# zju3dv/PVO

Hardware: AMD Instinct MI355X
Metric: VO keyframe updates/sec (8-keyframe window, 512x384, 36 edges; 6 graph updates + edge rebuild per keyframe) (higher is better)
Workload: dtype f16 (volume, lookup, update operator) / f32 (BA assembly) / f64 (pose solve); 1 GPU; S-B: BASELINE.json configs[1] window (8 keyframes, 48x64 maps, E=36, itrs=2), synthetic; edges=36, parallelism=independent window per GPU

## Files before the change

pvo_amd/csrc/conv_small.hip:

```cpp
#include "operand16.h"
#include <type_traits>
#include "glo_tile.h"
#include <stdlib.h>

namespace {

constexpr int kTH = 8, kTW = 16, kR = 3;
#ifndef PVO_CONV7_ROWS
#define PVO_CONV7_ROWS 16
#endif
constexpr int kTH7 = PVO_CONV7_ROWS;
constexpr int kHW_ = kTW + 2 * kR, kHH7 = kTH7 + 2 * kR;
constexpr int kTaps = 49, kSteps = 13;

template <typename T>
__global__ __launch_bounds__(256) void conv7x7_c8_kernel(const uint16_t* __restrict__ x, const uint16_t* __restrict__ wt,
                                                         const float* __restrict__ bias, uint16_t* __restrict__ y,
                                                         int H, int W) {
  __shared__ __attribute__((aligned(16))) unsigned char halo[kHH7 * kHW_ * 16];
  __shared__ __attribute__((aligned(16))) unsigned char slab[2][16 * 272];
  const int e = blockIdx.z, y0 = blockIdx.y * kTH7, x0 = blockIdx.x * kTW;
  const int tid = threadIdx.x, lane = tid & 63;
  const int wave = __builtin_amdgcn_readfirstlane(tid >> 6);
  const int li = lane & 15, lk = lane >> 4;
// ... 97 lines not shown
#pragma unroll
    for (int nt = 0; nt < NT; ++nt) bcur[kc][nt] = *reinterpret_cast<const u32x4*>(wl + static_cast<size_t>(nt) * 16 * 128 + kc * 32);
  v4f acc[kTH][NT];
#pragma unroll
  for (int py = 0; py < kTH; ++py)
#pragma unroll
    for (int nt = 0; nt < NT; ++nt) acc[py][nt] = v4f{0.f, 0.f, 0.f, 0.f};
  __syncthreads();

#pragma unroll 1
  for (int t = 0; t < 9; ++t) {
    if (t < 8) {
#pragma unroll
      for (int kc = 0; kc < 4; ++kc)
#pragma unroll
        for (int nt = 0; nt < NT; ++nt)
          bnxt[kc][nt] = *reinterpret_cast<const u32x4*>(wl + (t + 1) * tap_stride + static_cast<size_t>(nt) * 16 * 128 + kc * 32);
    }
    const unsigned char* tp = c3s + ((t / 3) * (kTW + 2) + (t % 3) + li) * kC3Stride + lk * 16;
#pragma unroll
    for (int py = 0; py < kTH; ++py) {
#pragma unroll
      for (int kc = 0; kc < 4; ++kc) {
        const u32x4 a = *reinterpret_cast<const u32x4*>(tp + py * (kTW + 2) * kC3Stride + kc * 64);
#pragma unroll
        for (int nt = 0; nt < NT; ++nt) acc[py][nt] = pvo_mfma<T>(a, bcur[kc][nt], acc[py][nt]);
      }
    }
    if (t < 8) {
#pragma unroll
      for (int kc = 0; kc < 4; ++kc)
#pragma unroll
        for (int nt = 0; nt < NT; ++nt) bcur[kc][nt] = bnxt[kc][nt];
    }
  }
  __syncthreads();
  constexpr int kOutStride = kCoutWG * 2 + 16;
  float bb[NT];
#pragma unroll
  for (int nt = 0; nt < NT; ++nt) bb[nt] = bias ? bias[co0 + nt * 16 + li] : 0.0f;
#pragma unroll
  for (int py = 0; py < kTH; ++py)
#pragma unroll
    for (int nt = 0; nt < NT; ++nt)
#pragma unroll
      for (int r = 0; r < 4; ++r) {
        float v = acc[py][nt][r] + bb[nt];
        if (relu) v = fmaxf(v, 0.0f);
        *reinterpret_cast<uint16_t*>(c3s + (py * 16 + lk * 4 + r) * kOutStride + (wave * 16 * NT + nt * 16 + li) * 2) =
            static_cast<uint16_t>(pvo_bits<T>(v));
      }
  __syncthreads();
  constexpr int kChunks = kCoutWG / 8;
  for (int id = tid; id < kTH * 16 * kChunks; id += 256) {
    const int p = id / kChunks, c = id - p * kChunks;
    const int gy = y0 + (p >> 4), gx = x0 + (p & 15);
    if (gy < H && gx < W)
      *reinterpret_cast<u32x4*>(y + ((static_cast<size_t>(e) * H + gy) * W + gx) * ystride + yoff + cg * kCoutWG + c * 8) =
          *reinterpret_cast<const u32x4*>(c3s + p * kOutStride + c * 16);
  }
}


struct BigEpi {
  int mode;
  const float* g;
  const uint16_t* P;
  const int* p_slots;
  const uint16_t* net;
  const uint16_t* Z;
  uint16_t* y2;
  int nseg;
  const uint16_t* seg_p[3]; int seg_stride[3]; int seg_chunks[3];
  const uint16_t* w2f;
  float* z;
};

constexpr int kBT = 16;
constexpr int kBHalo = (kBT + 2) * (kBT + 2);
constexpr int kBPitch = kBT + 2;
constexpr int kBStride = 96;
constexpr int kBA = 384 * kBStride;
constexpr int kBLds = 2 * kBA;

__device__ __forceinline__ int big_pix(int mt, int q) { return (q >> 1) * 16 + 2 * mt + (q & 1); }

#ifdef PVO_CONV_PROBE
__device__ unsigned long long* g_conv_probe = nullptr;
#define CONV_WG ((static_cast<size_t>(blockIdx.z) * gridDim.y + blockIdx.y) * gridDim.x + blockIdx.x)
#define CONV_PROBE(slot)                                                                                          \
  do {                                                                                                            \
    if (g_conv_probe && threadIdx.x == 0) g_conv_probe[CONV_WG * 8 + (slot)] = __builtin_readcyclecounter();      \
  } while (0)
#else
#define CONV_PROBE(slot)
#endif

template <typename T, bool HEADS>
__global__ __launch_bounds__(256, 2) void conv3x3_big_kernel(const uint16_t* __restrict__ x, const uint16_t* __restrict__ wt,
                                                          const float* __restrict__ bias, uint16_t* __restrict__ y,
                                                          int H, int W, int Cin, int Cout, int relu, int ystride, int yoff, BigEpi ep) {
  extern __shared__ __attribute__((aligned(16))) unsigned char bs[];
  unsigned char* As = bs;
  CONV_PROBE(0);
#ifdef PVO_CONV_PROBE
  if (g_conv_probe && threadIdx.x == 0) {
    g_conv_probe[CONV_WG * 8 + 4] = (static_cast<unsigned long long>(__builtin_amdgcn_s_getreg(20 | (31 << 11))) << 32) | __builtin_amdgcn_s_getreg(4 | (31 << 11));
    g_conv_probe[CONV_WG * 8 + 5] = wall_clock64();
  }
#endif
  const int ntx = (W + kBT - 1) / kBT;
  const int cg = blockIdx.x / ntx, tx_ = blockIdx.x - cg * ntx;
  const int e = blockIdx.z, y0 = blockIdx.y * kBT, x0 = tx_ * kBT;
  const int tid = threadIdx.x, lane = tid & 63;
  const int wave = __builtin_amdgcn_readfirstlane(tid >> 6);
  const int wm = wave >> 1, wn = wave & 1;
  const int li = lane & 15, kg = lane >> 4;
  const int nC = Cin >> 5;
  const uint16_t* xe = x + static_cast<size_t>(e) * H * W * Cin;

  u32x4 ra[3];
  int apix[6];
#pragma unroll
  for (int it = 0; it < 6; ++it) {
    const int id = tid + 256 * it;
    const int pos = id >> 2;
    apix[it] = -1;
    if (pos < kBHalo) {
      const int hr = pos / (kBT + 2), hc = pos % (kBT + 2);
      const int hy = y0 - 1 + hr, hx = x0 - 1 + hc;
      if (hy >= 0 && hy < H && hx >= 0 && hx < W) apix[it] = hy * W + hx;
    }
  }
  const int lpos0 = (tid >> 2) * kBStride + (tid & 3) * 16;
  auto lpos = [&](int it) { return lpos0 + it * 64 * kBStride; };
  const size_t img = static_cast<size_t>(e) * H * W;
  const uint16_t* a_src = xe; int a_stride = Cin, a_coff = 0;
  auto select_a = [&](int cc) {
    a_src = xe; a_stride = Cin; a_coff = cc * 32;
    if (ep.nseg > 0) {
      int sgi = 0, c0 = cc;
      while (sgi + 1 < ep.nseg && c0 >= ep.seg_chunks[sgi]) { c0 -= ep.seg_chunks[sgi]; ++sgi; }
      a_stride = ep.seg_stride[sgi];
      a_src = ep.seg_p[sgi] + img * a_stride;
      a_coff = c0 * 32;
    }
  };
  auto fetch_a = [&](int half) {
#pragma unroll
    for (int k = 0; k < 3; ++k)
      ra[k] = *reinterpret_cast<const u32x4*>(a_src + static_cast<size_t>(max(apix[3 * half + k], 0)) * a_stride + a_coff + (tid & 3) * 8);
  };
  auto store_a = [&](int buf, int half) {
#pragma unroll
    for (int k = 0; k < 3; ++k) {
      u32x4 v = ra[k];
      if (apix[3 * half + k] < 0) v = u32x4{0u, 0u, 0u, 0u};
      *reinterpret_cast<u32x4*>(As + buf * kBA + lpos(3 * half + k)) = v;
    }
  };

  float ginit[4] = {0.0f, 0.0f, 0.0f, 0.0f};
  if (!HEADS && ep.mode != 0) {
#pragma unroll
    for (int nt = 0; nt < 4; ++nt)
      ginit[nt] = ep.g[static_cast<size_t>(e) * 384 + (ep.mode == 1 ? cg * 128 : 256) + wn * 64 + nt * 16 + li];
  }
  v4f acc[8][4];
#pragma unroll
  for (int mt = 0; mt < 8; ++mt)
#pragma unroll
    for (int nt = 0; nt < 4; ++nt)
#pragma unroll
      for (int r = 0; r < 4; ++r) acc[mt][nt][r] = ginit[nt];

  const int S = nC * 9;
  {
    const uint16_t* wf = wt + (static_cast<size_t>(cg) * S * 8 + wn * 4) * 512;
    const int lane_off = lane * 8;
    u32x4 bset[3][4];
    auto fetch_bf = [&](u32x4 (&r)[4], int s) {
      const uint16_t* p = wf + static_cast<size_t>(min(s, S - 1)) * 4096;
#pragma unroll
      for (int f = 0; f < 4; ++f) r[f] = *reinterpret_cast<const u32x4*>(p + lane_off + f * 512);
    };
    select_a(0);
    {
      u32x4 r6[6];
#pragma unroll
      for (int k = 0; k < 6; ++k)
        r6[k] = *reinterpret_cast<const u32x4*>(a_src + static_cast<size_t>(max(apix[k], 0)) * a_stride + a_coff + (tid & 3) * 8);
      fetch_bf(bset[0], 0); fetch_bf(bset[1], 1);
#pragma unroll
      for (int k = 0; k < 6; ++k) {
        u32x4 v = r6[k];
        if (apix[k] < 0) v = u32x4{0u, 0u, 0u, 0u};
        *reinterpret_cast<u32x4*>(As + lpos(k)) = v;
      }
    }
    __syncthreads();
    CONV_PROBE(1);
    const unsigned char* Abase = As + ((8 * wm + (li >> 1)) * kBPitch + (li & 1)) * kBStride + kg * 16;
    auto main_loop = [&](auto nh_c) {
    constexpr int NH = decltype(nh_c)::value;
    auto read_half = [&](u32x4 (&a)[4], const unsigned char* Ac, int toff, int h) {
#pragma unroll
      for (int i = 0; i < 4; ++i) a[i] = *reinterpret_cast<const u32x4*>(Ac + toff + (4 * h + i) * 2 * kBStride);
    };
    auto mfma_half = [&](const u32x4 (&a)[4], const u32x4 (&bf)[4], int h, bool n_major) {
#pragma unroll
      for (int j = 0; j < 16; ++j) {
        const int i = n_major ? (j & 3) : (j >> 2), nt = n_major ? (j >> 2) : (j & 3);
        acc[4 * h + i][nt] = pvo_mfma<T>(a[i], bf[nt], acc[4 * h + i][nt]);
      }
    };
    auto pin_reads_b = [&]() {
#pragma unroll
      for (int i = 0; i < 4; ++i) {
        __builtin_amdgcn_sched_group_barrier(0x8, 1, 0); __builtin_amdgcn_sched_group_barrier(0x100, 1, 0);
        __builtin_amdgcn_sched_group_barrier(0x8, 1, 0); __builtin_amdgcn_sched_group_barrier(0x20, 1, 0);
      }
    };
    auto pin_reads = [&]() {
#pragma unroll
      for (int i = 0; i < 4; ++i) { __builtin_amdgcn_sched_group_barrier(0x8, 2, 0); __builtin_amdgcn_sched_group_barrier(0x100, 1, 0); }
    };
    auto pin_staging = [&](int t) {
      if (t == 3 || t == 7) {
#pragma unroll
        for (int i = 0; i < 3; ++i) { __builtin_amdgcn_sched_group_barrier(0x8, 1, 0); __builtin_amdgcn_sched_group_barrier(0x200, 1, 0); }
      }
      if (t == 3) { __builtin_amdgcn_sched_group_barrier(0x8, 1, 0); __builtin_amdgcn_sched_group_barrier(0x20, 3, 0); }
    };
#pragma unroll 1
    for (int cc = 0; cc < nC; ++cc) {
      const unsigned char* Ac = Abase + (cc & 1) * kBA;
      select_a(min(cc + 1, nC - 1));
      fetch_a(0);
      u32x4 a0[4], a1[4];
      read_half(a0, Ac, 0, 0);
      __builtin_amdgcn_sched_barrier(0);
#pragma unroll
      for (int t = 0; t < 9; ++t) {
        const int toff = ((t / 3) * kBPitch + (t % 3)) * kBStride;
        const int toff1 = (((t + 1) / 3) * kBPitch + ((t + 1) % 3)) * kBStride;
        fetch_bf(bset[(t + 2) % 3], cc * 9 + t + 2);
        const u32x4 (&bf)[4] = bset[t % 3];
        if (NH == 2) {
          read_half(a1, Ac, toff, 1);
          mfma_half(a0, bf, 0, false);
          pin_reads_b();
          __builtin_amdgcn_sched_barrier(0);
          if (t < 8) read_half(a0, Ac, toff1, 0);
          if (t == 3) { store_a((cc + 1) & 1, 0); fetch_a(1); }
          if (t == 7) store_a((cc + 1) & 1, 1);
          mfma_half(a1, bf, 1, true);
          if (t < 8) pin_reads();
          pin_staging(t);
        } else {
          u32x4 (&cur)[4] = (t & 1) ? a1 : a0;
          u32x4 (&nxt)[4] = (t & 1) ? a0 : a1;
          if (t < 8) read_half(nxt, Ac, toff1, 0);
          if (t == 3) { store_a((cc + 1) & 1, 0); fetch_a(1); }
          if (t == 7) store_a((cc + 1) & 1, 1);
          mfma_half(cur, bf, 0, true);
          if (t < 8) pin_reads_b();
          else {
#pragma unroll
            for (int i = 0; i < 4; ++i) { __builtin_amdgcn_sched_group_barrier(0x8, 1, 0); __builtin_amdgcn_sched_group_barrier(0x20, 1, 0); }
          }
          pin_staging(t);
        }
        __builtin_amdgcn_sched_barrier(0);
      }
      __syncthreads();
    }
    };
    if (x0 + 8 >= W) main_loop(std::integral_constant<int, 1>{});
    else main_loop(std::integral_constant<int, 2>{});
  }
  CONV_PROBE(2);

  if (!HEADS && ep.mode != 0) {
    float* slab = reinterpret_cast<float*>(bs);
    const int c = tid & 15, m0 = tid >> 4;
    const int pstride = ep.mode == 1 ? 256 : 128;
    const uint16_t* gate_p = ep.P + (ep.mode == 1 ? cg * 128 : 0) + c * 8;
    uint16_t* const dst = (ep.mode == 1 && cg != 0) ? ep.y2 : y;
    const int ep_ = ep.p_slots ? ep.p_slots[e] : e;
    u32x4 pv[4], nv[4], zv[4];
    auto request = [&](int half, int b) {
#pragma unroll
      for (int k = 0; k < 4; ++k) {
        const int m = m0 + 16 * (4 * b + k);
        const int gy = y0 + 8 * half + (m >> 4), gx = x0 + (m & 15);
        const bool in = gy < H && gx < W;
        const size_t rr = in ? (static_cast<size_t>(e) * H + gy) * W + gx : 0;
        const size_t rp = in ? (static_cast<size_t>(ep_) * H + gy) * W + gx : 0;
        pv[k] = *reinterpret_cast<const u32x4*>(gate_p + rp * pstride);
        nv[k] = *reinterpret_cast<const u32x4*>(ep.net + rr * 128 + c * 8);
        if (ep.mode == 2) zv[k] = *reinterpret_cast<const u32x4*>(ep.Z + rr * 128 + c * 8);
      }
    };
    auto finish = [&](int half, int b) {
#pragma unroll
      for (int k = 0; k < 4; ++k) {
        const int m = m0 + 16 * (4 * b + k);
        const int gy = y0 + 8 * half + (m >> 4), gx = x0 + (m & 15);
        float a[8], pp[8], nn[8], o[8];
        const float4 a0 = *reinterpret_cast<const float4*>(slab + m * 132 + c * 8), a1 = *reinterpret_cast<const float4*>(slab + m * 132 + c * 8 + 4);
        a[0] = a0.x; a[1] = a0.y; a[2] = a0.z; a[3] = a0.w; a[4] = a1.x; a[5] = a1.y; a[6] = a1.z; a[7] = a1.w;
        pvo_unpack8<T>(pv[k], pp);
        pvo_unpack8<T>(nv[k], nn);
        if (ep.mode == 1) {
#pragma unroll
          for (int q = 0; q < 8; ++q) o[q] = __builtin_amdgcn_rcpf(1.0f + __builtin_amdgcn_exp2f(-1.4426950408889634f * (a[q] + pp[q])));
          if (cg != 0) {
#pragma unroll
            for (int q = 0; q < 8; ++q) o[q] *= nn[q];
          }
        } else {
          float zz[8];
          pvo_unpack8<T>(zv[k], zz);
#pragma unroll
          for (int q = 0; q < 8; ++q) {
            const float th = 1.0f - 2.0f * __builtin_amdgcn_rcpf(1.0f + __builtin_amdgcn_exp2f(2.8853900817779268f * (a[q] + pp[q])));
            o[q] = (1.0f - zz[q]) * nn[q] + zz[q] * th;
          }
        }
        if (gy < H && gx < W) *reinterpret_cast<u32x4*>(dst + ((static_cast<size_t>(e) * H + gy) * W + gx) * 128 + c * 8) = pvo_pack8<T>(o);
      }
    };
#pragma unroll 1
    for (int half = 0; half < 2; ++half) {
      request(half, 0);
      if (wm == half) {
#pragma unroll
        for (int mt = 0; mt < 8; ++mt)
#pragma unroll
          for (int nt = 0; nt < 4; ++nt)
#pragma unroll
            for (int r = 0; r < 4; ++r) slab[big_pix(mt, 4 * kg + r) * 132 + wn * 64 + nt * 16 + li] = acc[mt][nt][r];
      }
      __syncthreads();
      if (half == 0) CONV_PROBE(6);
      finish(half, 0);
      request(half, 1);
      finish(half, 1);
      __syncthreads();
      if (half == 0) CONV_PROBE(7);
    }
    CONV_PROBE(3);
    return;
  }
  float bb[4];
#pragma unroll
  for (int nt = 0; nt < 4; ++nt) bb[nt] = bias ? bias[cg * 128 + wn * 64 + nt * 16 + li] : 0.0f;
  unsigned char* w2s = bs + 36 * 1024;
  if (HEADS) {
    const u32x4* src = reinterpret_cast<const u32x4*>(ep.w2f + static_cast<size_t>(cg) * 4096) + tid;
    const u32x4 f0 = src[0], f1 = src[256];
    *reinterpret_cast<u32x4*>(w2s + tid * 16) = f0;
    *reinterpret_cast<u32x4*>(w2s + 4096 + tid * 16) = f1;
  }
#pragma unroll 1
  for (int half = 0; half < 2; ++half) {
    if (wm == half) {
#pragma unroll
      for (int mt = 0; mt < 8; ++mt)
#pragma unroll
        for (int nt = 0; nt < 4; ++nt)
#pragma unroll
          for (int r = 0; r < 4; ++r) {
            const int m = big_pix(mt, 4 * kg + r);
            float v = acc[mt][nt][r] + bb[nt];
            if (relu) v = fmaxf(v, 0.0f);
            *reinterpret_cast<uint16_t*>(bs + m * 272 + (wn * 64 + nt * 16 + li) * 2) = static_cast<uint16_t>(pvo_bits<T>(v));
          }
    }
    __syncthreads();
    if (HEADS) {
      v16f zz;
#pragma unroll
      for (int r = 0; r < 16; ++r) zz[r] = 0.0f;
      const int l32 = lane & 31, k32 = lane >> 5;
      const unsigned char* arow = bs + (32 * wave + l32) * 272 + k32 * 16;
#pragma unroll
      for (int ks = 0; ks < 8; ++ks)
        zz = pvo_mfma32<T>(*reinterpret_cast<const u32x4*>(arow + ks * 32), *reinterpret_cast<const u32x4*>(w2s + (ks * 64 + lane) * 16), zz);
      if (l32 < 18) {
#pragma unroll
        for (int r = 0; r < 16; ++r) {
          const int m = 32 * wave + (r & 3) + 8 * (r >> 2) + 4 * k32;
          const int gy = y0 + 8 * half + (m >> 4), gx = x0 + (m & 15);
          if (gy < H && gx < W) ep.z[(((static_cast<size_t>(e) * H + gy) * W + gx) * (Cout >> 7) + cg) * 18 + l32] = zz[r];
        }
      }
    } else {
      for (int id = tid; id < 128 * 16; id += 256) {
        const int m = id >> 4, c = id & 15;
        const int gy = y0 + 8 * half + (m >> 4), gx = x0 + (m & 15);
        if (gy < H && gx < W)
          *reinterpret_cast<u32x4*>(y + ((static_cast<size_t>(e) * H + gy) * W + gx) * ystride + yoff + cg * 128 + c * 8) =
              *reinterpret_cast<const u32x4*>(bs + m * 272 + c * 16);
      }
    }
    __syncthreads();
  }
  CONV_PROBE(3);
}

constexpr int kFeOW = 14;
constexpr int kFeRows = kTH + 2;
constexpr int kFeM7W = 16 + 2 * kR;
constexpr int kFeM7Pos = (kFeRows + 2 * kR) * kFeM7W;
constexpr int kFeF1Pos = kFeRows * 16 + 2;
constexpr int kFeLds = kFeF1Pos * kC3Stride + kFeM7Pos * 16;

template <typename T>
__global__ __launch_bounds__(256) void flow_encoder_kernel(const uint16_t* __restrict__ x, const uint16_t* __restrict__ w7,
                                                           const float* __restrict__ b7, const uint16_t* __restrict__ w3,
                                                           const float* __restrict__ b3, uint16_t* __restrict__ y,
                                                           int H, int W, int ystride, int yoff) {
  extern __shared__ __attribute__((aligned(16))) unsigned char fes[];
  unsigned char* f1 = fes;
  unsigned char* halo = fes + kFeF1Pos * kC3Stride;
  const int e = blockIdx.z, y0 = blockIdx.y * kTH, x0 = blockIdx.x * kFeOW;
  const int tid = threadIdx.x, lane = tid & 63;
  const int wave = __builtin_amdgcn_readfirstlane(tid >> 6);
  const int li = lane & 15, lk = lane >> 4;

  {
    u32x4 bf[kSteps][2];
#pragma unroll
    for (int s = 0; s < kSteps; ++s)
#pragma unroll
      for (int nt = 0; nt < 2; ++nt)
        bf[s][nt] = *reinterpret_cast<const u32x4*>(w7 + (static_cast<size_t>(4 * s + lk) * 128 + wave * 32 + nt * 16 + li) * 8);
    const uint16_t* xe = x + static_cast<size_t>(e) * H * W * 8;
    for (int pos = tid; pos < kFeM7Pos; pos += 256) {
      const int hy = y0 - 1 - kR + pos / kFeM7W, hx = x0 - 1 - kR + pos % kFeM7W;
      u32x4 v = {0u, 0u, 0u, 0u};
      if (hy >= 0 && hy < H && hx >= 0 && hx < W) v = *reinterpret_cast<const u32x4*>(xe + (static_cast<size_t>(hy) * W + hx) * 8);
      *reinterpret_cast<u32x4*>(halo + pos * 16) = v;
    }
    if (tid < 2 * 17) *reinterpret_cast<u32x4*>(f1 + kFeRows * 16 * kC3Stride + tid * 16) = u32x4{0u, 0u, 0u, 0u};
    int toff[kSteps];
#pragma unroll
    for (int s = 0; s < kSteps; ++s) {
      const int tap = min(4 * s + lk, kTaps - 1);
      toff[s] = ((tap / 7) * kFeM7W + (tap % 7) + li) * 16;
    }
    const float bb0 = b7[wave * 32 + li], bb1 = b7[wave * 32 + 16 + li];
    __syncthreads();
    for (int r = 0; r < kFeRows; ++r) {
      const int gy = y0 - 1 + r;
      v4f d0 = {0.f, 0.f, 0.f, 0.f}, d1 = {0.f, 0.f, 0.f, 0.f};
      const bool row_in = gy >= 0 && gy < H;
      if (row_in) {
        const unsigned char* rowp = halo + r * kFeM7W * 16;
        u32x4 afr[kSteps];
#pragma unroll
        for (int s = 0; s < kSteps; ++s) afr[s] = *reinterpret_cast<const u32x4*>(rowp + toff[s]);
#pragma unroll
        for (int s = 0; s < kSteps; ++s) {
          d0 = pvo_mfma<T>(afr[s], bf[s][0], d0);
          d1 = pvo_mfma<T>(afr[s], bf[s][1], d1);
        }
      }
#pragma unroll
      for (int q = 0; q < 4; ++q) {
        const int p = lk * 4 + q, gx = x0 - 1 + p;
        const bool in = row_in && gx >= 0 && gx < W;
        unsigned char* dst = f1 + (r * 16 + p) * kC3Stride + (wave * 32 + li) * 2;
        *reinterpret_cast<uint16_t*>(dst) = in ? static_cast<uint16_t>(pvo_bits<T>(fmaxf(d0[q] + bb0, 0.0f))) : static_cast<uint16_t>(0);
        *reinterpret_cast<uint16_t*>(dst + 32) = in ? static_cast<uint16_t>(pvo_bits<T>(fmaxf(d1[q] + bb1, 0.0f))) : static_cast<uint16_t>(0);
      }
    }
  }
  const int co0 = wave * 16;
  const uint16_t* wl = w3 + (static_cast<size_t>(co0 + li)) * 128 + lk * 8;
  constexpr size_t tap_stride = static_cast<size_t>(64) * 128;
  u32x4 bcur[4], bnxt[4];
#pragma unroll
  for (int kc = 0; kc < 4; ++kc) bcur[kc] = *reinterpret_cast<const u32x4*>(wl + kc * 32);
  v4f acc[kTH];
#pragma unroll
  for (int py = 0; py < kTH; ++py) acc[py] = v4f{0.f, 0.f, 0.f, 0.f};
  __syncthreads();
#pragma unroll 1
// ... 62 lines not shown

extern "C" int pvo_flow_encoder(const void* x, const void* w7_taps, const float* bias7, const void* w3_taps, const float* bias3,
                                void* y, int E, int H, int W, int ystride, int yoff, int dtype, void* stream) {
  if (E < 0 || H < 0 || W < 0) return PVO_EINVAL;
  if (ystride == 0) ystride = 64;
  if (ystride < yoff + 64 || yoff < 0 || (ystride & 7) || (yoff & 7)) return PVO_EINVAL;
  if (E == 0 || H == 0 || W == 0) return PVO_OK;
  if (!x || !w7_taps || !bias7 || !w3_taps || !y || E > 65535) return PVO_EINVAL;
  if (pvo_misaligned16(x, w7_taps, w3_taps, y)) return PVO_EINVAL;
  hipStream_t st = pvo_stream(stream);
  const dim3 grid((W + kFeOW - 1) / kFeOW, (H + kTH - 1) / kTH, E);
  const uint16_t *xp = static_cast<const uint16_t*>(x), *w7 = static_cast<const uint16_t*>(w7_taps), *w3 = static_cast<const uint16_t*>(w3_taps);
  return pvo_dispatch16(dtype, [&](auto tag) -> int {
    using T = decltype(tag);
    if (!pvo_allow_lds<flow_encoder_kernel<T>>(kFeLds)) return PVO_ELAUNCH;
    hipLaunchKernelGGL(flow_encoder_kernel<T>, grid, dim3(256), kFeLds, st, xp, w7, bias7, w3, bias3, static_cast<uint16_t*>(y), H, W, ystride, yoff);
    PVO_CHECK_LAUNCH();
    return PVO_OK;
  });
}

extern "C" int pvo_gru_glo_chunks(int HW) { return HW <= 0 ? 0 : (HW + 255) / 256; }

extern "C" int pvo_gru_glo_fused(const void* net, const void* w_weight, const float* w_bias, float* glo_part,
                                 int E, int HW, int dtype, void* stream) {
  if (E < 0 || HW < 0) return PVO_EINVAL;
  if (E == 0 || HW == 0) return PVO_OK;
  if (!net || !w_weight || !glo_part || E > 65535) return PVO_EINVAL;
  if (pvo_misaligned16(net, w_weight)) return PVO_EINVAL;
  hipStream_t st = pvo_stream(stream);
  const int chunk = 256;
  dim3 grid(pvo_gru_glo_chunks(HW), E);
  return pvo_dispatch16(dtype, [&](auto tag) -> int {
    using T = decltype(tag);
    hipLaunchKernelGGL(gru_glo_mfma_kernel<T>, grid, dim3(256), 0, st, static_cast<const uint16_t*>(net),
                       static_cast<const uint16_t*>(w_weight), w_bias, glo_part, HW, chunk);
    PVO_CHECK_LAUNCH();
    return PVO_OK;
  });
}

extern "C" int pvo_conv3x3_c128(const void* x, const void* w_taps, const float* bias, void* y,
                                int E, int H, int W, int Cout, int relu, int ystride, int yoff, int dtype, void* stream) {
  if (E < 0 || H < 0 || W < 0) return PVO_EINVAL;
  if (Cout != 64 && (Cout <= 0 || (Cout & 127))) return PVO_EUNSUPPORTED;
  if (ystride == 0) ystride = Cout;
  if (ystride < yoff + Cout || yoff < 0 || (ystride & 7) || (yoff & 7)) return PVO_EINVAL;
  if (E == 0 || H == 0 || W == 0) return PVO_OK;
  if (!x || !w_taps || !y || E > 65535) return PVO_EINVAL;
  if (pvo_misaligned16(x, w_taps, y)) return PVO_EINVAL;
  hipStream_t st = pvo_stream(stream);
  const int ntx = (W + kTW - 1) / kTW;
  const size_t lds = static_cast<size_t>(kC3Halo) * kC3Stride;
  const uint16_t* xp = static_cast<const uint16_t*>(x);
  const uint16_t* wp = static_cast<const uint16_t*>(w_taps);
  uint16_t* yp = static_cast<uint16_t*>(y);
  return pvo_dispatch16(dtype, [&](auto tag) -> int {
    using T = decltype(tag);
    if (Cout == 64) {
      dim3 grid(ntx, (H + kTH - 1) / kTH, E);
      hipLaunchKernelGGL((conv3x3_c128_kernel<T, 1>), grid, dim3(256), lds, st, xp, wp, bias, yp, H, W, Cout, relu, ystride, yoff);
    } else {
      dim3 grid(ntx * (Cout / 128), (H + kTH - 1) / kTH, E);
      hipLaunchKernelGGL((conv3x3_c128_kernel<T, 2>), grid, dim3(256), lds, st, xp, wp, bias, yp, H, W, Cout, relu, ystride, yoff);
    }
    PVO_CHECK_LAUNCH();
    return PVO_OK;
  });
}

static int launch_big(const void* x, const void* w_taps, const float* bias, void* y,
                      int E, int H, int W, int Cin, int Cout, int relu, int ystride, int yoff, int dtype, void* stream,
                      const BigEpi& ep) {
  if (E < 0 || H < 0 || W < 0) return PVO_EINVAL;
  if (Cin <= 0 || (Cin & 31) || Cout <= 0 || (Cout & 127)) return PVO_EUNSUPPORTED;
  if (ystride == 0) ystride = Cout;
  if (ystride < yoff + Cout || yoff < 0 || (ystride & 7) || (yoff & 7)) return PVO_EINVAL;
  if (E == 0 || H == 0 || W == 0) return PVO_OK;
  if (!x || !w_taps || !y || E > 65535) return PVO_EINVAL;
  if (pvo_misaligned16(x, w_taps, y)) return PVO_EINVAL;
  if (static_cast<long long>(H) * W * Cin > 0x7fffffffLL) return PVO_EUNSUPPORTED;
  hipStream_t st = pvo_stream(stream);
  const int ntx = (W + kBT - 1) / kBT;
  const size_t lds = kBLds;
  dim3 grid(ntx * (Cout / 128), (H + kBT - 1) / kBT, E);
  const uint16_t* xp = static_cast<const uint16_t*>(x);
  const uint16_t* wp = static_cast<const uint16_t*>(w_taps);
  uint16_t* yp = static_cast<uint16_t*>(y);
  return pvo_dispatch16(dtype, [&](auto tag) -> int {
    using T = decltype(tag);
    if (ep.mode == 3) {
      if (!pvo_allow_lds<conv3x3_big_kernel<T, true>>(lds)) return PVO_ELAUNCH;
      hipLaunchKernelGGL((conv3x3_big_kernel<T, true>), grid, dim3(256), lds, st, xp, wp, bias, yp, H, W, Cin, Cout, relu, ystride, yoff, ep);
    } else {
      if (!pvo_allow_lds<conv3x3_big_kernel<T, false>>(lds)) return PVO_ELAUNCH;
      hipLaunchKernelGGL((conv3x3_big_kernel<T, false>), grid, dim3(256), lds, st, xp, wp, bias, yp, H, W, Cin, Cout, relu, ystride, yoff, ep);
    }
    PVO_CHECK_LAUNCH();
    return PVO_OK;
  });
}

extern "C" int pvo_conv3x3(const void* x, const void* w_taps, const float* bias, void* y,
                           int E, int H, int W, int Cin, int Cout, int relu, int ystride, int yoff, int dtype, void* stream) {
  return launch_big(x, w_taps, bias, y, E, H, W, Cin, Cout, relu, ystride, yoff, dtype, stream, BigEpi{});
}

extern "C" int pvo_conv3x3_heads(const void* x, const void* w1_taps, const float* bias1, const void* w2_frags, float* z,
                                 int E, int H, int W, int dtype, void* stream) {
  if (!bias1 || !w2_frags || !z || pvo_misaligned16(w2_frags)) return PVO_EINVAL;
  BigEpi ep{};
  ep.mode = 3; ep.w2f = static_cast<const uint16_t*>(w2_frags); ep.z = z;
  return launch_big(x, w1_taps, bias1, z, E, H, W, 128, 512, 1, 0, 0, dtype, stream, ep);
}

static int seg_setup(BigEpi& ep, const void* first, const void* cf, int cf_channels) {
  if (!first || !cf) return PVO_EINVAL;
  if (pvo_misaligned16(first, cf)) return PVO_EINVAL;
  if (cf_channels <= 0 || (cf_channels & 31)) return PVO_EUNSUPPORTED;
  ep.nseg = 2;
  ep.seg_p[0] = static_cast<const uint16_t*>(first); ep.seg_stride[0] = 128; ep.seg_chunks[0] = 4;
  ep.seg_p[1] = static_cast<const uint16_t*>(cf); ep.seg_stride[1] = cf_channels; ep.seg_chunks[1] = cf_channels >> 5;
  return PVO_OK;
}

extern "C" int pvo_gru_conv_gates(const void* net, const void* cf, int cf_channels, const void* w_taps, const float* g,
                                  const void* P_zr, const int* p_slots, void* Z, void* RN, int E, int H, int W, int dtype, void* stream) {
  if (!g || !P_zr || !RN) return PVO_EINVAL;
  if (pvo_misaligned16(P_zr, RN)) return PVO_EINVAL;
  BigEpi ep{};
  const int rc = seg_setup(ep, net, cf, cf_channels);
  if (rc != PVO_OK) return rc;
  ep.mode = 1; ep.g = g; ep.P = static_cast<const uint16_t*>(P_zr); ep.p_slots = p_slots; ep.net = static_cast<const uint16_t*>(net);
  ep.y2 = static_cast<uint16_t*>(RN);
  return launch_big(net, w_taps, nullptr, Z, E, H, W, 128 + cf_channels, 256, 0, 0, 0, dtype, stream, ep);
}

extern "C" int pvo_gru_conv_candidate(const void* RN, const void* cf, int cf_channels, const void* w_taps, const float* g,
                                      const void* P_q, const int* p_slots, const void* Z, const void* net, void* net_out,
                                      int E, int H, int W, int dtype, void* stream) {
  if (!g || !P_q || !net || !Z) return PVO_EINVAL;
  if (pvo_misaligned16(P_q, net, Z)) return PVO_EINVAL;
  BigEpi ep{};
  const int rc = seg_setup(ep, RN, cf, cf_channels);
  if (rc != PVO_OK) return rc;
  ep.mode = 2; ep.g = g; ep.P = static_cast<const uint16_t*>(P_q); ep.p_slots = p_slots; ep.net = static_cast<const uint16_t*>(net);
  ep.Z = static_cast<const uint16_t*>(Z);
  return launch_big(RN, w_taps, nullptr, net_out, E, H, W, 128 + cf_channels, 128, 0, 0, 0, dtype, stream, ep);
}
```

pvo_amd/droid_backends.py:

```python
import ctypes
import itertools

import torch

from . import _lib
from ._lib import PvoHipError, check

_DT = {torch.float32: _lib.PVO_F32, torch.float16: _lib.PVO_F16,
       torch.bfloat16: _lib.PVO_BF16, torch.float64: _lib.PVO_F64}

_ws_cache = {}


def _contig(t, name):
    if not t.is_contiguous():
        raise RuntimeError("%s must be contiguous" % name)


def _dev(*ts):
    dev = None
    for t in ts:
        if t is None:
            continue
        if not t.is_cuda:
# ... 571 lines not shown
    if b is None:
        return ctypes.c_void_p(0)
    if b.dtype != torch.float32 or b.numel() != C or not b.is_contiguous() or not b.is_cuda:
        raise PvoHipError("%s must be a contiguous float32 device vector of %d elements" % (what, C))
    return _ptr(b)


def _new_cl(E, C, H, W, dtype, dev):
    return torch.empty(E, H, W, C, dtype=dtype, device=dev).permute(0, 3, 1, 2)


def gru_glo_fused(net, w_weight, w_bias=None):
    _cl(net, "net", 128)
    dev = _dev(net, w_weight)
    E, C, H, W = net.shape
    w2d = w_weight.reshape(128, 128)
    if w2d.dtype != net.dtype or not w2d.is_contiguous():
        raise PvoHipError("gru_glo_fused: w_weight must be a contiguous [128,128] tensor in net's dtype")
    lib = _lib.load()
    part = torch.empty(E, lib.pvo_gru_glo_chunks(H * W), C, dtype=torch.float32, device=dev)
    with torch.cuda.device(dev):
        check(lib.pvo_gru_glo_fused(_ptr(net), _ptr(w2d), _bias(w_bias, C, "w_bias"), _ptr(part), E, H * W,
                                    _dtype_code(net, "net"), _stream(dev)), "gru_glo_fused")
    return part


def gate_context(glo_part, wg_t, g_bias):
    dev = _dev(glo_part, wg_t, g_bias)
    E, K, C = glo_part.shape
    for t, n in ((glo_part, "glo_part"), (wg_t, "wg_t"), (g_bias, "g_bias")):
        _f32(t, n); _contig(t, n)
    if C != 128 or tuple(wg_t.shape) != (128, 384) or g_bias.numel() != 384:
        raise PvoHipError("gate_context: glo_part [E,K,128], wg_t [128,384], g_bias [384]")
    g = torch.empty(E, 384, dtype=torch.float32, device=dev)
    with torch.cuda.device(dev):
        check(_lib.load().pvo_gate_context(_ptr(glo_part), _ptr(wg_t), _ptr(g_bias), _ptr(g), E, K, _stream(dev)), "gate_context")
    return g


def conv7x7_c8_weights(weight, dtype):
    co, ci, kh, kw = weight.shape
    if (co, ci, kh, kw) != (128, 8, 7, 7):
        raise PvoHipError("conv7x7_c8: filter must be [128,8,7,7]")
    w = torch.zeros(52, 128, 8, dtype=dtype, device=weight.device)
    w[:49] = weight.detach().permute(2, 3, 0, 1).reshape(49, 128, 8).to(dtype)
    return w.contiguous()


def conv7x7_c8(x, w_taps, bias):
    _cl(x, "x", 8)
    dev = _dev(x, w_taps, bias)
    E, _, H, W = x.shape
    if w_taps.dtype != x.dtype or tuple(w_taps.shape) != (52, 128, 8) or not w_taps.is_contiguous():
        raise PvoHipError("conv7x7_c8: w_taps must be the [52,128,8] tensor of conv7x7_c8_weights in x's dtype")
    y = _new_cl(E, 128, H, W, x.dtype, dev)
    with torch.cuda.device(dev):
        check(_lib.load().pvo_conv7x7_c8(_ptr(x), _ptr(w_taps), _bias(bias, 128, "bias"), _ptr(y), E, H, W,
                                         _dtype_code(x, "x"), _stream(dev)), "conv7x7_c8")
    return y


def flow_encoder(x, w7_taps, bias7, w3_taps, bias3, out=None, out_offset=0):
    _cl(x, "x", 8)
    dev = _dev(x, w7_taps, bias7, w3_taps, out)
    E, _, H, W = x.shape
    if w7_taps.dtype != x.dtype or tuple(w7_taps.shape) != (52, 128, 8) or not w7_taps.is_contiguous():
        raise PvoHipError("flow_encoder: w7_taps must be the [52,128,8] tensor of conv7x7_c8_weights in x's dtype")
    if tuple(w3_taps.shape) != (9, 64, 128) or w3_taps.dtype != x.dtype or not w3_taps.is_contiguous():
        raise PvoHipError("flow_encoder: w3_taps must be the [9,64,128] tensor of conv3x3_c128_weights in x's dtype")
    ret, y, ys, yo = _out_slice(out, out_offset, E, 64, H, W, x.dtype, dev)
    with torch.cuda.device(dev):
        check(_lib.load().pvo_flow_encoder(_ptr(x), _ptr(w7_taps), _bias(bias7, 128, "bias7"), _ptr(w3_taps), _bias(bias3, 64, "bias3"),
                                           _ptr(y), E, H, W, ys, yo, _dtype_code(x, "x"), _stream(dev)), "flow_encoder")
    return ret


def conv3x3_c128_weights(weight, dtype):
    co, ci, kh, kw = weight.shape
    if (kh, kw) != (3, 3):
        raise PvoHipError("conv3x3: filter must be [Cout,Cin,3,3]")
    return weight.detach().permute(2, 3, 0, 1).reshape(9, co, ci).to(dtype).contiguous()


def conv3x3_weights(weight, dtype):
    co, ci, kh, kw = weight.shape
    if (kh, kw) != (3, 3) or ci % 32 or co % 128:
        raise PvoHipError("conv3x3: filter must be [Cout,Cin,3,3] with Cin % 32 == 0 and Cout % 128 == 0")
    taps = weight.detach().permute(2, 3, 0, 1).reshape(9, co, ci).to(dtype)
    f = taps.reshape(9, co // 128, 2, 4, 16, ci // 32, 4, 8).permute(1, 5, 0, 2, 3, 6, 4, 7)
    return f.contiguous().view(9, co, ci)


def _out_slice(out, out_offset, E, Cout, H, W, dtype, dev):
    if out is None:
        y = _new_cl(E, Cout, H, W, dtype, dev)
        return y, y, 0, 0
    if out.dim() != 4 or out.shape[0] != E or tuple(out.shape[2:]) != (H, W) or out.dtype != dtype or \
            not out.is_contiguous(memory_format=torch.channels_last) or out_offset < 0 or out_offset + Cout > out.shape[1]:
        raise PvoHipError("out must be a channels-last [E,C>=offset+Cout,H,W] tensor of the input dtype")
    return out[:, out_offset:out_offset + Cout], out, out.shape[1], out_offset


def conv3x3(x, w_taps, bias=None, relu=False, out=None, out_offset=0):
    dev = _dev(x, w_taps, out)
    E, Cin, H, W = x.shape
    _cl(x, "x", Cin)
    if w_taps.dim() != 3 or w_taps.shape[0] != 9 or w_taps.shape[2] != Cin or w_taps.dtype != x.dtype or not w_taps.is_contiguous():
        raise PvoHipError("conv3x3: w_taps must be the [9,Cout,Cin] tensor of conv3x3_weights in x's dtype")
    Cout = w_taps.shape[1]
    ret, y, ys, yo = _out_slice(out, out_offset, E, Cout, H, W, x.dtype, dev)
    with torch.cuda.device(dev):
        check(_lib.load().pvo_conv3x3(_ptr(x), _ptr(w_taps), _bias(bias, Cout, "bias"), _ptr(y), E, H, W, Cin, Cout,
                                      1 if relu else 0, ys, yo, _dtype_code(x, "x"), _stream(dev)), "conv3x3")
    return ret


def conv3x3_c128(x, w_taps, bias=None, relu=False, out=None, out_offset=0):
    _cl(x, "x", 128)
    dev = _dev(x, w_taps, out)
    E, _, H, W = x.shape
    if w_taps.dim() != 3 or w_taps.shape[0] != 9 or w_taps.shape[2] != 128 or w_taps.dtype != x.dtype or not w_taps.is_contiguous():
        raise PvoHipError("conv3x3_c128: w_taps must be the [9,Cout,128] tensor of conv3x3_weights in x's dtype")
    Cout = w_taps.shape[1]
    ret, y, ys, yo = _out_slice(out, out_offset, E, Cout, H, W, x.dtype, dev)
    with torch.cuda.device(dev):
        check(_lib.load().pvo_conv3x3_c128(_ptr(x), _ptr(w_taps), _bias(bias, Cout, "bias"), _ptr(y), E, H, W, Cout,
                                           1 if relu else 0, ys, yo, _dtype_code(x, "x"), _stream(dev)), "conv3x3_c128")
    return ret


def gru_conv_gates(net, cf, w_taps, g, P_zr, p_slots=None):
    E, _, H, W = net.shape
    C = cf.shape[1]
    _cl(net, "net", 128); _cl(cf, "cf", C); _cl(P_zr, "P_zr", 256)
    dev = _dev(net, cf, w_taps, g, P_zr, p_slots)
    if p_slots is not None and (p_slots.dtype != torch.int32 or p_slots.numel() != E or not p_slots.is_contiguous()):
        raise PvoHipError("gru_conv_gates: p_slots must be a contiguous int32 [E] tensor")
    _f32(g, "g"); _contig(g, "g")
    if tuple(w_taps.shape) != (9, 256, 128 + C) or w_taps.dtype != net.dtype or not w_taps.is_contiguous():
        raise PvoHipError("gru_conv_gates: w_taps must be [9,256,128+C] in net's dtype")
    Z, RN = _new_cl(E, 128, H, W, net.dtype, dev), _new_cl(E, 128, H, W, net.dtype, dev)
    with torch.cuda.device(dev):
        check(_lib.load().pvo_gru_conv_gates(_ptr(net), _ptr(cf), C, _ptr(w_taps), _ptr(g), _ptr(P_zr), _vp(p_slots), _ptr(Z), _ptr(RN),
                                             E, H, W, _dtype_code(net, "net"), _stream(dev)), "gru_conv_gates")
    return Z, RN


def gru_conv_candidate(RN, cf, w_taps, g, P_q, Z, net, p_slots=None):
    E, _, H, W = net.shape
    C = cf.shape[1]
    _cl(RN, "RN", 128); _cl(cf, "cf", C); _cl(P_q, "P_q", 128); _cl(Z, "Z", 128); _cl(net, "net", 128)
    dev = _dev(RN, cf, w_taps, g, P_q, Z, net)
    _f32(g, "g"); _contig(g, "g")
    if tuple(w_taps.shape) != (9, 128, 128 + C) or w_taps.dtype != net.dtype or not w_taps.is_contiguous():
        raise PvoHipError("gru_conv_candidate: w_taps must be [9,128,128+C] in net's dtype")
    out = _new_cl(E, 128, H, W, net.dtype, dev)
    with torch.cuda.device(dev):
        check(_lib.load().pvo_gru_conv_candidate(_ptr(RN), _ptr(cf), C, _ptr(w_taps), _ptr(g), _ptr(P_q), _vp(p_slots), _ptr(Z), _ptr(net),
                                                 _ptr(out), E, H, W, _dtype_code(net, "net"), _stream(dev)), "gru_conv_candidate")
    return out


def corr_encode(corr, enc_weight, enc_bias):
    _cl(corr, "corr", 196)
    dev = _dev(corr, enc_weight, enc_bias)
    E, _, H, W = corr.shape
    if tuple(enc_weight.shape) != (128, 224) or enc_weight.dtype != corr.dtype or not enc_weight.is_contiguous():
        raise PvoHipError("enc_weight must be the [128,224] tensor of corr_encoder_weights in the feature dtype")
    y = _new_cl(E, 128, H, W, corr.dtype, dev)
    with torch.cuda.device(dev):
        check(_lib.load().pvo_corr_encode(_ptr(corr), _ptr(enc_weight), _bias(enc_bias, 128, "enc_bias"), _ptr(y), E * H * W,
                                          _dtype_code(corr, "corr"), _stream(dev)), "corr_encode")
# ... 730 lines not shown
```

Measured before the change: 252.6 keyframe updates/s.

## Transpose MFMA operands in big conv so epilogues write straight from registers

Swaps the A/B operands of the MFMA in the 3x3 big conv and reorders the packed weight layout so each lane's accumulators hold 8 consecutive output channels of one pixel. The gated GRU epilogue and the plain bias/relu store can then pack and write directly from registers, with no LDS slab round-trip and no syncthreads. The heads path still stages through LDS, but over the whole tile in one pass with a larger LDS allocation and vectorised z stores. The risks are the larger LDS footprint for heads, which limits occupancy, and less coalesced global stores of 64 bytes per lane.

```diff
diff --git a/pvo_amd/csrc/conv_small.hip b/pvo_amd/csrc/conv_small.hip
--- a/pvo_amd/csrc/conv_small.hip
+++ b/pvo_amd/csrc/conv_small.hip
@@ -203,8 +203,13 @@
 constexpr int kBStride = 96;
 constexpr int kBA = 384 * kBStride;
 constexpr int kBLds = 2 * kBA;
+constexpr int kBSlab = 256 * 272;
+constexpr int kBLdsHeads = kBSlab + 8192;
+static_assert(kBLdsHeads >= kBLds && 2 * kBLdsHeads <= 160 * 1024, "the heads' slab must cover the halo and leave room for two workgroups");
 
 __device__ __forceinline__ int big_pix(int mt, int q) { return (q >> 1) * 16 + 2 * mt + (q & 1); }
+__device__ __forceinline__ int big_chan(int nt, int kg) { return 32 * (nt >> 1) + 8 * kg + 4 * (nt & 1); }
+struct __attribute__((packed, aligned(8))) BigZ4 { float v[4]; };
 
 #ifdef PVO_CONV_PROBE
 __device__ unsigned long long* g_conv_probe = nullptr;
@@ -281,19 +286,25 @@
     }
   };
 
-  float ginit[4] = {0.0f, 0.0f, 0.0f, 0.0f};
-  if (!HEADS && ep.mode != 0) {
+  v4f acc[8][4];
+  {
+    v4f ginit[4];
 #pragma unroll
     for (int nt = 0; nt < 4; ++nt)
-      ginit[nt] = ep.g[static_cast<size_t>(e) * 384 + (ep.mode == 1 ? cg * 128 : 256) + wn * 64 + nt * 16 + li];
-  }
-  v4f acc[8][4];
-#pragma unroll
-  for (int mt = 0; mt < 8; ++mt)
-#pragma unroll
-    for (int nt = 0; nt < 4; ++nt)
-#pragma unroll
-      for (int r = 0; r < 4; ++r) acc[mt][nt][r] = ginit[nt];
+#pragma unroll
+      for (int r = 0; r < 4; ++r) ginit[nt][r] = 0.0f;
+    if (!HEADS && ep.mode != 0) {
+      const float* gp = ep.g + static_cast<size_t>(e) * 384 + (ep.mode == 1 ? cg * 128 : 256) + wn * 64;
+#pragma unroll
+      for (int nt = 0; nt < 4; ++nt)
+#pragma unroll
+        for (int r = 0; r < 4; ++r) ginit[nt][r] = gp[big_chan(nt, kg) + r];
+    }
+#pragma unroll
+    for (int mt = 0; mt < 8; ++mt)
+#pragma unroll
+      for (int nt = 0; nt < 4; ++nt) acc[mt][nt] = ginit[nt];
+  }
 
   const int S = nC * 9;
   {
@@ -332,7 +343,7 @@
 #pragma unroll
       for (int j = 0; j < 16; ++j) {
         const int i = n_major ? (j & 3) : (j >> 2), nt = n_major ? (j >> 2) : (j & 3);
-        acc[4 * h + i][nt] = pvo_mfma<T>(a[i], bf[nt], acc[4 * h + i][nt]);
+        acc[4 * h + i][nt] = pvo_mfma<T>(bf[nt], a[i], acc[4 * h + i][nt]);
       }
     };
     auto pin_reads_b = [&]() {
@@ -402,37 +413,46 @@
   }
   CONV_PROBE(2);
 
+  const int elane = __builtin_amdgcn_mbcnt_hi(~0u, __builtin_amdgcn_mbcnt_lo(~0u, 0u));
+  const int etid = wave * 64 + elane, eli = elane & 15, ekg = elane >> 4;
+  const bool nh1 = x0 + 8 >= W;
+  const int gy = y0 + 8 * wm + (eli >> 1), gx0 = x0 + (eli & 1);
+  const int cb = wn * 64 + ekg * 8;
+  auto gather8 = [&](int mt, int h, float a[8]) {
+#pragma unroll
+    for (int q = 0; q < 8; ++q) a[q] = acc[mt][2 * h + (q >> 2)][q & 3];
+  };
+
   if (!HEADS && ep.mode != 0) {
-    float* slab = reinterpret_cast<float*>(bs);
-    const int c = tid & 15, m0 = tid >> 4;
     const int pstride = ep.mode == 1 ? 256 : 128;
-    const uint16_t* gate_p = ep.P + (ep.mode == 1 ? cg * 128 : 0) + c * 8;
-    uint16_t* const dst = (ep.mode == 1 && cg != 0) ? ep.y2 : y;
+    const uint16_t* gate_p = ep.P + (ep.mode == 1 ? cg * 128 : 0) + cb;
+    const uint16_t* net_p = ep.net + cb;
+    const uint16_t* z_p = ep.mode == 2 ? ep.Z + cb : net_p;
+    uint16_t* const dst = ((ep.mode == 1 && cg != 0) ? ep.y2 : y) + cb;
     const int ep_ = ep.p_slots ? ep.p_slots[e] : e;
-    u32x4 pv[4], nv[4], zv[4];
-    auto request = [&](int half, int b) {
-#pragma unroll
-      for (int k = 0; k < 4; ++k) {
-        const int m = m0 + 16 * (4 * b + k);
-        const int gy = y0 + 8 * half + (m >> 4), gx = x0 + (m & 15);
-        const bool in = gy < H && gx < W;
-        const size_t rr = in ? (static_cast<size_t>(e) * H + gy) * W + gx : 0;
-        const size_t rp = in ? (static_cast<size_t>(ep_) * H + gy) * W + gx : 0;
-        pv[k] = *reinterpret_cast<const u32x4*>(gate_p + rp * pstride);
-        nv[k] = *reinterpret_cast<const u32x4*>(ep.net + rr * 128 + c * 8);
-        if (ep.mode == 2) zv[k] = *reinterpret_cast<const u32x4*>(ep.Z + rr * 128 + c * 8);
-      }
-    };
-    auto finish = [&](int half, int b) {
-#pragma unroll
-      for (int k = 0; k < 4; ++k) {
-        const int m = m0 + 16 * (4 * b + k);
-        const int gy = y0 + 8 * half + (m >> 4), gx = x0 + (m & 15);
+    u32x4 pv[2][2], nv[2][2], zv[2][2];
+    auto request = [&](int mt, int s) {
+      const int gx = gx0 + 2 * mt;
+      const bool in = gy < H && gx < W;
+      const size_t rr = in ? (static_cast<size_t>(e) * H + gy) * W + gx : 0;
+      const size_t rp = in ? (static_cast<size_t>(ep_) * H + gy) * W + gx : 0;
+#pragma unroll
+      for (int h = 0; h < 2; ++h) {
+        pv[s][h] = *reinterpret_cast<const u32x4*>(gate_p + rp * pstride + 32 * h);
+        nv[s][h] = *reinterpret_cast<const u32x4*>(net_p + rr * 128 + 32 * h);
+        if (ep.mode == 2) zv[s][h] = *reinterpret_cast<const u32x4*>(z_p + rr * 128 + 32 * h);
+      }
+    };
+    auto finish = [&](int mt, int s) {
+      const int gx = gx0 + 2 * mt;
+      const bool in = gy < H && gx < W;
+      uint16_t* const d = dst + ((static_cast<size_t>(e) * H + gy) * W + gx) * 128;
+#pragma unroll
+      for (int h = 0; h < 2; ++h) {
         float a[8], pp[8], nn[8], o[8];
-        const float4 a0 = *reinterpret_cast<const float4*>(slab + m * 132 + c * 8), a1 = *reinterpret_cast<const float4*>(slab + m * 132 + c * 8 + 4);
-        a[0] = a0.x; a[1] = a0.y; a[2] = a0.z; a[3] = a0.w; a[4] = a1.x; a[5] = a1.y; a[6] = a1.z; a[7] = a1.w;
-        pvo_unpack8<T>(pv[k], pp);
-        pvo_unpack8<T>(nv[k], nn);
+        gather8(mt, h, a);
+        pvo_unpack8<T>(pv[s][h], pp);
+        pvo_unpack8<T>(nv[s][h], nn);
         if (ep.mode == 1) {
 #pragma unroll
           for (int q = 0; q < 8; ++q) o[q] = __builtin_amdgcn_rcpf(1.0f + __builtin_amdgcn_exp2f(-1.4426950408889634f * (a[q] + pp[q])));
@@ -442,91 +462,126 @@
           }
         } else {
           float zz[8];
-          pvo_unpack8<T>(zv[k], zz);
+          pvo_unpack8<T>(zv[s][h], zz);
 #pragma unroll
           for (int q = 0; q < 8; ++q) {
             const float th = 1.0f - 2.0f * __builtin_amdgcn_rcpf(1.0f + __builtin_amdgcn_exp2f(2.8853900817779268f * (a[q] + pp[q])));
             o[q] = (1.0f - zz[q]) * nn[q] + zz[q] * th;
           }
         }
-        if (gy < H && gx < W) *reinterpret_cast<u32x4*>(dst + ((static_cast<size_t>(e) * H + gy) * W + gx) * 128 + c * 8) = pvo_pack8<T>(o);
-      }
-    };
-#pragma unroll 1
-    for (int half = 0; half < 2; ++half) {
-      request(half, 0);
-      if (wm == half) {
-#pragma unroll
-        for (int mt = 0; mt < 8; ++mt)
-#pragma unroll
-          for (int nt = 0; nt < 4; ++nt)
-#pragma unroll
-            for (int r = 0; r < 4; ++r) slab[big_pix(mt, 4 * kg + r) * 132 + wn * 64 + nt * 16 + li] = acc[mt][nt][r];
-      }
-      __syncthreads();
-      if (half == 0) CONV_PROBE(6);
-      finish(half, 0);
-      request(half, 1);
-      finish(half, 1);
-      __syncthreads();
-      if (half == 0) CONV_PROBE(7);
+        if (in) *reinterpret_cast<u32x4*>(d + 32 * h) = pvo_pack8<T>(o);
+      }
+    };
+    request(0, 0);
+#pragma unroll
+    for (int mt = 0; mt < 4; ++mt) {
+      request(mt + 1, (mt + 1) & 1);
+      finish(mt, mt & 1);
+      if (mt == 0) CONV_PROBE(6);
+    }
+    CONV_PROBE(7);
+    if (!nh1) {
+#pragma unroll
+      for (int mt = 4; mt < 8; ++mt) {
+        if (mt < 7) request(mt + 1, (mt + 1) & 1);
+        finish(mt, mt & 1);
+      }
     }
     CONV_PROBE(3);
     return;
   }
-  float bb[4];
-#pragma unroll
-  for (int nt = 0; nt < 4; ++nt) bb[nt] = bias ? bias[cg * 128 + wn * 64 + nt * 16 + li] : 0.0f;
-  unsigned char* w2s = bs + 36 * 1024;
-  if (HEADS) {
-    const u32x4* src = reinterpret_cast<const u32x4*>(ep.w2f + static_cast<size_t>(cg) * 4096) + tid;
+
+  float bb[4][4];
+#pragma unroll
+  for (int nt = 0; nt < 4; ++nt)
+#pragma unroll
+    for (int r = 0; r < 4; ++r) bb[nt][r] = 0.0f;
+  if (HEADS || bias) {
+    const float* const bp = bias + cg * 128 + wn * 64;
+#pragma unroll
+    for (int nt = 0; nt < 4; ++nt)
+#pragma unroll
+      for (int r = 0; r < 4; ++r) bb[nt][r] = bp[big_chan(nt, ekg) + r];
+  }
+  auto act8 = [&](int mt, int h, float o[8]) {
+    gather8(mt, h, o);
+#pragma unroll
+    for (int q = 0; q < 8; ++q) {
+      o[q] += bb[2 * h + (q >> 2)][q & 3];
+      if (relu) o[q] = fmaxf(o[q], 0.0f);
+    }
+  };
+
+  if (!HEADS) {
+    uint16_t* const yb = y + yoff + cg * 128 + cb;
+    auto store_tile = [&](int mt) {
+      const int gx = gx0 + 2 * mt;
+      if (gy < H && gx < W) {
+        uint16_t* const d = yb + ((static_cast<size_t>(e) * H + gy) * W + gx) * ystride;
+#pragma unroll
+        for (int h = 0; h < 2; ++h) {
+          float o[8];
+          act8(mt, h, o);
+          *reinterpret_cast<u32x4*>(d + 32 * h) = pvo_pack8<T>(o);
+        }
+      }
+    };
+#pragma unroll
+    for (int mt = 0; mt < 4; ++mt) {
+      store_tile(mt);
+      if (mt == 0) CONV_PROBE(6);
+    }
+    CONV_PROBE(7);
+    if (!nh1) {
+#pragma unroll
+      for (int mt = 4; mt < 8; ++mt) store_tile(mt);
+    }
+    CONV_PROBE(3);
+    return;
+  }
+
+  unsigned char* w2s = bs + kBSlab;
+  {
+    const u32x4* src = reinterpret_cast<const u32x4*>(ep.w2f + static_cast<size_t>(cg) * 4096) + etid;
     const u32x4 f0 = src[0], f1 = src[256];
-    *reinterpret_cast<u32x4*>(w2s + tid * 16) = f0;
-    *reinterpret_cast<u32x4*>(w2s + 4096 + tid * 16) = f1;
-  }
-#pragma unroll 1
-  for (int half = 0; half < 2; ++half) {
-    if (wm == half) {
-#pragma unroll
-      for (int mt = 0; mt < 8; ++mt)
-#pragma unroll
-        for (int nt = 0; nt < 4; ++nt)
-#pragma unroll
-          for (int r = 0; r < 4; ++r) {
-            const int m = big_pix(mt, 4 * kg + r);
-            float v = acc[mt][nt][r] + bb[nt];
-            if (relu) v = fmaxf(v, 0.0f);
-            *reinterpret_cast<uint16_t*>(bs + m * 272 + (wn * 64 + nt * 16 + li) * 2) = static_cast<uint16_t>(pvo_bits<T>(v));
-          }
-    }
-    __syncthreads();
-    if (HEADS) {
+    *reinterpret_cast<u32x4*>(w2s + etid * 16) = f0;
+    *reinterpret_cast<u32x4*>(w2s + 4096 + etid * 16) = f1;
+  }
+  {
+    unsigned char* const hrow = bs + (128 * wm + eli) * 272 + cb * 2;
+#pragma unroll
+    for (int mt = 0; mt < 8; ++mt)
+#pragma unroll
+      for (int h = 0; h < 2; ++h) {
+        float o[8];
+        act8(mt, h, o);
+        *reinterpret_cast<u32x4*>(hrow + mt * 16 * 272 + h * 64) = pvo_pack8<T>(o);
+      }
+  }
+  __syncthreads();
+  CONV_PROBE(6);
+  if (!(nh1 && (wave & 1))) {
+    const int l32 = elane & 31, k32 = elane >> 5;
+#pragma unroll
+    for (int b = 0; b < 2; ++b) {
+      const int R = 64 * wave + 32 * b + l32;
       v16f zz;
 #pragma unroll
       for (int r = 0; r < 16; ++r) zz[r] = 0.0f;
-      const int l32 = lane & 31, k32 = lane >> 5;
-      const unsigned char* arow = bs + (32 * wave + l32) * 272 + k32 * 16;
+      const unsigned char* hr = bs + R * 272 + k32 * 16;
 #pragma unroll
       for (int ks = 0; ks < 8; ++ks)
-        zz = pvo_mfma32<T>(*reinterpret_cast<const u32x4*>(arow + ks * 32), *reinterpret_cast<const u32x4*>(w2s + (ks * 64 + lane) * 16), zz);
-      if (l32 < 18) {
-#pragma unroll
-        for (int r = 0; r < 16; ++r) {
-          const int m = 32 * wave + (r & 3) + 8 * (r >> 2) + 4 * k32;
-          const int gy = y0 + 8 * half + (m >> 4), gx = x0 + (m & 15);
-          if (gy < H && gx < W) ep.z[(((static_cast<size_t>(e) * H + gy) * W + gx) * (Cout >> 7) + cg) * 18 + l32] = zz[r];
-        }
-      }
-    } else {
-      for (int id = tid; id < 128 * 16; id += 256) {
-        const int m = id >> 4, c = id & 15;
-        const int gy = y0 + 8 * half + (m >> 4), gx = x0 + (m & 15);
-        if (gy < H && gx < W)
-          *reinterpret_cast<u32x4*>(y + ((static_cast<size_t>(e) * H + gy) * W + gx) * ystride + yoff + cg * 128 + c * 8) =
-              *reinterpret_cast<const u32x4*>(bs + m * 272 + c * 16);
-      }
-    }
-    __syncthreads();
+        zz = pvo_mfma32<T>(*reinterpret_cast<const u32x4*>(w2s + (ks * 64 + elane) * 16), *reinterpret_cast<const u32x4*>(hr + ks * 32), zz);
+      if (b == 1) CONV_PROBE(7);
+      const int zy = y0 + 8 * (R >> 7) + ((R & 15) >> 1), zx = x0 + 2 * ((R >> 4) & 7) + (R & 1);
+      if (zy < H && zx < W) {
+        float* const zp = ep.z + (((static_cast<size_t>(e) * H + zy) * W + zx) * (Cout >> 7) + cg) * 18;
+#pragma unroll
+        for (int g = 0; g < 2; ++g)
+          *reinterpret_cast<BigZ4*>(zp + 8 * g + 4 * k32) = BigZ4{{zz[4 * g], zz[4 * g + 1], zz[4 * g + 2], zz[4 * g + 3]}};
+        if (k32 == 0) *reinterpret_cast<float2*>(zp + 16) = make_float2(zz[8], zz[9]);
+      }
+    }
   }
   CONV_PROBE(3);
 }
@@ -755,7 +810,7 @@
   if (static_cast<long long>(H) * W * Cin > 0x7fffffffLL) return PVO_EUNSUPPORTED;
   hipStream_t st = pvo_stream(stream);
   const int ntx = (W + kBT - 1) / kBT;
-  const size_t lds = kBLds;
+  const size_t lds = ep.mode == 3 ? kBLdsHeads : kBLds;
   dim3 grid(ntx * (Cout / 128), (H + kBT - 1) / kBT, E);
   const uint16_t* xp = static_cast<const uint16_t*>(x);
   const uint16_t* wp = static_cast<const uint16_t*>(w_taps);
diff --git a/pvo_amd/droid_backends.py b/pvo_amd/droid_backends.py
--- a/pvo_amd/droid_backends.py
+++ b/pvo_amd/droid_backends.py
@@ -677,12 +677,15 @@
     return weight.detach().permute(2, 3, 0, 1).reshape(9, co, ci).to(dtype).contiguous()
 
 
+WIDE_CONV_CHANNEL_SPLIT = (2, 2, 4, 2, 4)
+
+
 def conv3x3_weights(weight, dtype):
     co, ci, kh, kw = weight.shape
     if (kh, kw) != (3, 3) or ci % 32 or co % 128:
         raise PvoHipError("conv3x3: filter must be [Cout,Cin,3,3] with Cin % 32 == 0 and Cout % 128 == 0")
     taps = weight.detach().permute(2, 3, 0, 1).reshape(9, co, ci).to(dtype)
-    f = taps.reshape(9, co // 128, 2, 4, 16, ci // 32, 4, 8).permute(1, 5, 0, 2, 3, 6, 4, 7)
+    f = taps.reshape((9, co // 128) + WIDE_CONV_CHANNEL_SPLIT + (ci // 32, 4, 8)).permute(1, 7, 0, 2, 3, 5, 8, 4, 6, 9)
     return f.contiguous().view(9, co, ci)
 
 
```

Result: no change. 251.7 keyframe updates/s (-0.3%).
